# Artemarius/cuda-gaussian-splatting

Hardware: AMD Instinct MI355X
Metric: fwd+bwd Mpixels/s @1080p, 1M Gaussians, SH3 (higher is better)
Workload: dtype f32

## Files before the change

### cuda-gaussian-splatting_amd/csrc/cugs_raster_common.h

```cpp
#pragma once

#include "cugs_gaussian_math.h"

#define CUGS_REC_F4 3

struct RasterGeom {
    int width, height, ntx, ntiles;
    float bg0, bg1, bg2;
};

struct RasterSrc {
    const int32_t* tile_ranges;
    const int32_t* gidx;
    const float* packed;
    const float* means_2d;
    const float* cov_2d_inv;
    const float* rgb;
    const float* opa;
    const uint4* tile_order;
};

template <bool PACKED, bool DEPTH = false>
__device__ __forceinline__ int stage_record(const RasterSrc& s, int li, int end, float4* s_rec,
                                            const float* __restrict__ depths = nullptr) {
    if (li >= end) return -1;
    const int g = s.gidx[li];
    float4 r0, r1, r2;
    if (PACKED) {
        const float4* src = reinterpret_cast<const float4*>(s.packed + (int64_t)g * CUGS_PACKED_STRIDE);
        r0 = src[0]; r1 = src[1]; r2 = src[2];
    } else {
        const float a = s.cov_2d_inv[g * 3 + 0], c = s.cov_2d_inv[g * 3 + 2], o = s.opa[g];
        r0 = make_float4(s.means_2d[g * 2 + 0], s.means_2d[g * 2 + 1], a, s.cov_2d_inv[g * 3 + 1]);
        r1 = make_float4(c, o, (o >= (1.0f / 255.0f)) ? logf(255.0f * o) : -1.0f, 0.0f);
        r2 = make_float4(s.rgb[g * 3 + 0], 0.0f, s.rgb[g * 3 + 1], s.rgb[g * 3 + 2]);
    }
    r1.w = __int_as_float(g);
    if (DEPTH) r2.y = depths[g];
    s_rec[threadIdx.x * CUGS_REC_F4 + 0] = r0;
    s_rec[threadIdx.x * CUGS_REC_F4 + 1] = r1;
    s_rec[threadIdx.x * CUGS_REC_F4 + 2] = r2;
    return g;
}

__device__ __forceinline__ bool may_touch_quad(float4 r0, float4 r1, float qx0, float qy0,
                                               float wx, float wy) {
    const float mx = r0.x, my = r0.y, a = r0.z, b = r0.w, c = r1.x;
    const float tau = r1.z;
    if (!(tau >= 0.0f)) return false;
    if (!(a > 0.0f && c > 0.0f)) return true;
    const float ia = __builtin_amdgcn_rcpf(a), ic = __builtin_amdgcn_rcpf(c);
    const float lx = qx0 - mx, hx = lx + wx, ly = qy0 - my, hy = ly + wy;
    const bool inside = (lx <= 0.0f) && (hx >= 0.0f) && (ly <= 0.0f) && (hy >= 0.0f);
    float X, Y;
    asm("v_max_f32_e64 %0, -%1, %2" : "=v"(X) : "v"(lx), "v"(hx));
    asm("v_max_f32_e64 %0, -%1, %2" : "=v"(Y) : "v"(ly), "v"(hy));
    const float B = a * X * X + 2.0f * fabsf(b) * X * Y + c * Y * Y;
    const float b2 = b + b;
    const float xe = (lx > 0.0f) ? lx : hx, ye = (ly > 0.0f) ? ly : hy;
    const float yv = __builtin_amdgcn_fmed3f(-b * xe * ic, ly, hy);
    const float xv = __builtin_amdgcn_fmed3f(-b * ye * ia, lx, hx);
    const float qx = a * xe * xe + b2 * xe * yv + c * yv * yv;
    const float qy = a * xv * xv + b2 * xv * ye + c * ye * ye;
    const bool out_x = !((lx <= 0.0f) && (hx >= 0.0f)), out_y = !((ly <= 0.0f) && (hy >= 0.0f));
    const float qmin = inside ? 0.0f : fminf(out_x ? qx : 3.0e38f, out_y ? qy : 3.0e38f);
    return !(0.5f * qmin > tau * 1.01f + 0.05f + 4e-6f * B);
}

struct ActiveRect { float x0, y0, wx, wy; };
__device__ __forceinline__ ActiveRect active_rect(unsigned long long active, float quad_cx, float quad_cy) {
    unsigned cols = (unsigned)active | (unsigned)(active >> 32);
    cols |= cols >> 16;
    cols |= cols >> 8;
    cols &= 0xFFu;
    const int x0 = __builtin_ctz(cols), x1 = 31 - __builtin_clz(cols);
    const int y0 = __builtin_ctzll(active) >> 3, y1 = (63 - __builtin_clzll(active)) >> 3;
    return ActiveRect{quad_cx + (float)x0, quad_cy + (float)y0, (float)(x1 - x0), (float)(y1 - y0)};
}

struct PixelEval { float dx, dy, gx, gy, e; };
__device__ __forceinline__ float pixel_alpha_raw(float pxf, float pyf, float mx, float my, float a, float b,
                                                 float c, float o, float open, PixelEval& r) {
    r.dx = pxf - mx;
    r.dy = pyf - my;
    r.gx = fmaf(a, r.dx, b * r.dy);
    r.gy = fmaf(b, r.dx, c * r.dy);
    const float q = fmaf(r.dx, r.gx, r.dy * r.gy);
    r.e = cugs_blend_exp_q(q);
    const float gate = fmaf(q, 0x1p127f, 1.0f);
    return __builtin_fminf(__builtin_fminf((o * open) * r.e, 0.99f), gate);
}
__device__ __forceinline__ float pixel_alpha(float pxf, float pyf, float mx, float my, float a, float b,
                                             float c, float o, float open, PixelEval& r) {
    const float alpha = pixel_alpha_raw(pxf, pyf, mx, my, a, b, c, o, open, r);
    return (alpha < (1.0f / 255.0f)) ? 0.0f : alpha;
}


__device__ __forceinline__ float sat_fma(float a, float b, float c) {
    return __builtin_amdgcn_fmed3f(fmaf(a, b, c), 0.0f, 1.0f);
}
__device__ __forceinline__ float sat_add(float a, float b) { return __builtin_amdgcn_fmed3f(a + b, 0.0f, 1.0f); }

#define CUGS_ALPHA_MIN_PRED 0x1.01010p-8f
__device__ __forceinline__ float passes_alpha_min(float x) {
    return sat_fma(x, 0x1p32f, -CUGS_ALPHA_MIN_PRED * 0x1p32f);
}
__device__ __forceinline__ float below_alpha_cap(float x) { return sat_fma(x, -0x1p32f, 0.99f * 0x1p32f); }

__device__ __forceinline__ int reduce9t_slot(int lane) {
    if (lane & 3) return -1;
    const int bank = (lane >> 2) & 3, row = lane >> 4;
    const int perm[4] = {0, 2, 1, 3};
    if (row == 0) return perm[bank];
    if (row == 1) return bank == 3 ? 8 : 4 + perm[bank];
    if (row == 2 && bank == 0) return 7;
    return -1;
}

__device__ __forceinline__ float reduce9t(float cA, float cB, float v2, float v3, float v4, float v5, float v6,
                                          float v8, float v7) {
    float a0, a1, a2, a3, a4, b0, b1, b2, d;
    asm volatile(
        "s_nop 1\n\t"
        "v_add_f32_dpp %0, %10, %9 row_mirror row_mask:0xf bank_mask:0xf\n\t"
        "v_add_f32_dpp %1, %11, %11 row_mirror row_mask:0xf bank_mask:0x3\n\t"
        "v_add_f32_dpp %1, %12, %12 row_mirror row_mask:0xf bank_mask:0xc\n\t"
        "v_add_f32_dpp %2, %13, %13 row_mirror row_mask:0xf bank_mask:0x3\n\t"
        "v_add_f32_dpp %2, %14, %14 row_mirror row_mask:0xf bank_mask:0xc\n\t"
        "v_add_f32_dpp %3, %15, %15 row_mirror row_mask:0xf bank_mask:0x3\n\t"
        "v_add_f32_dpp %3, %16, %16 row_mirror row_mask:0xf bank_mask:0xc\n\t"
        "v_add_f32_dpp %4, %17, %17 row_mirror row_mask:0xf bank_mask:0xf\n\t"
        "v_add_f32_dpp %5, %0, %0 row_half_mirror row_mask:0xf bank_mask:0x5\n\t"
        "v_add_f32_dpp %5, %1, %1 row_half_mirror row_mask:0xf bank_mask:0xa\n\t"
        "v_add_f32_dpp %7, %4, %4 row_half_mirror row_mask:0xf bank_mask:0xf\n\t"
        "v_add_f32_dpp %6, %2, %2 row_half_mirror row_mask:0xf bank_mask:0x5\n\t"
        "v_add_f32_dpp %6, %3, %3 row_half_mirror row_mask:0xf bank_mask:0xa\n\t"
        "v_mov_b32 %8, %7\n\t"
        "s_nop 1\n\t"
        "v_permlane16_swap_b32 %5, %6\n\t"
        "v_permlane16_swap_b32 %7, %8\n\t"
        "v_add_f32 %5, %5, %6\n\t"
        "v_add_f32 %7, %7, %8\n\t"
        "s_nop 1\n\t"
        "v_permlane32_swap_b32 %5, %7\n\t"
        "v_add_f32 %8, %5, %7\n\t"
        "s_nop 1\n\t"
        "v_add_f32_dpp %8, %8, %8 quad_perm:[1,0,3,2] row_mask:0xf bank_mask:0xf\n\t"
        "s_nop 1\n\t"
        "v_add_f32_dpp %8, %8, %8 quad_perm:[2,3,0,1] row_mask:0xf bank_mask:0xf\n\t"
        : "=&v"(a0), "=&v"(a1), "=&v"(a2), "=&v"(a3), "=&v"(a4), "=&v"(b0), "=&v"(b1), "=&v"(b2), "=&v"(d)
        : "v"(cA), "v"(cB), "v"(v2), "v"(v3), "v"(v4), "v"(v5), "v"(v6), "v"(v8), "v"(v7));
    return d;
}

template <int CTRL>
__device__ __forceinline__ float dpp_mov(float v) {
    return __builtin_bit_cast(float, __builtin_amdgcn_update_dpp(0, __builtin_bit_cast(int, v), CTRL, 0xF, 0xF, false));
}
template <int CTRL>
__device__ __forceinline__ float xchg_add(bool side, float a, float b) {
    return (side ? b : a) + dpp_mov<CTRL>(side ? a : b);
}

__device__ __forceinline__ int reduce9r16_slot(int lane) {
    const int r = lane & 15, bank = r >> 2;
    const int perm[4] = {0, 2, 1, 3};
    if ((r & 3) == 0) return perm[bank];
    if ((r & 3) == 2) return bank == 3 ? 8 : 4 + perm[bank];
    if (r == 1) return 7;
    return -1;
}

__device__ __forceinline__ float reduce_r16_tail(float b0, float b1, float b2, int lane) {
    const bool s1 = (lane & 2) != 0, s0 = (lane & 1) != 0;
    const float c0 = xchg_add<0x4E>(s1, b0, b1);
    const float c1 = b2 + dpp_mov<0x4E>(b2);
    return xchg_add<0xB1>(s0, c0, c1);
}

__device__ __forceinline__ float reduce9r16(float cA, float cB, float v2, float v3, float v4, float v5, float v6,
                                            float v8, float v7, int lane) {
    float a0, a1, a2, a3, a4, b0, b1, b2;
    asm volatile(
        "s_nop 1\n\t"
        "v_add_f32_dpp %0, %9, %8 row_mirror row_mask:0xf bank_mask:0xf\n\t"
        "v_add_f32_dpp %1, %10, %10 row_mirror row_mask:0xf bank_mask:0x3\n\t"
        "v_add_f32_dpp %1, %11, %11 row_mirror row_mask:0xf bank_mask:0xc\n\t"
        "v_add_f32_dpp %2, %12, %12 row_mirror row_mask:0xf bank_mask:0x3\n\t"
        "v_add_f32_dpp %2, %13, %13 row_mirror row_mask:0xf bank_mask:0xc\n\t"
        "v_add_f32_dpp %3, %14, %14 row_mirror row_mask:0xf bank_mask:0x3\n\t"
        "v_add_f32_dpp %3, %15, %15 row_mirror row_mask:0xf bank_mask:0xc\n\t"
        "v_add_f32_dpp %4, %16, %16 row_mirror row_mask:0xf bank_mask:0xf\n\t"
        "v_add_f32_dpp %5, %0, %0 row_half_mirror row_mask:0xf bank_mask:0x5\n\t"
        "v_add_f32_dpp %5, %1, %1 row_half_mirror row_mask:0xf bank_mask:0xa\n\t"
        "v_add_f32_dpp %7, %4, %4 row_half_mirror row_mask:0xf bank_mask:0xf\n\t"
        "v_add_f32_dpp %6, %2, %2 row_half_mirror row_mask:0xf bank_mask:0x5\n\t"
        "v_add_f32_dpp %6, %3, %3 row_half_mirror row_mask:0xf bank_mask:0xa\n\t"
        "s_nop 1\n\t"
        : "=&v"(a0), "=&v"(a1), "=&v"(a2), "=&v"(a3), "=&v"(a4), "=&v"(b0), "=&v"(b1), "=&v"(b2)
        : "v"(cA), "v"(cB), "v"(v2), "v"(v3), "v"(v4), "v"(v5), "v"(v6), "v"(v8), "v"(v7));
    return reduce_r16_tail(b0, b1, b2, lane);
}

__device__ __forceinline__ int reduce10r16_slot(int lane) {
    return ((lane & 15) == 9) ? 9 : reduce9r16_slot(lane);
}

__device__ __forceinline__ float reduce10r16(float cA, float cB, float v2, float v3, float v4, float v5, float v6,
                                             float v8, float v7, float v9, int lane) {
    float a0, a1, a2, a3, a4, b0, b1, b2;
    asm volatile(
        "s_nop 1\n\t"
        "v_add_f32_dpp %0, %9, %8 row_mirror row_mask:0xf bank_mask:0xf\n\t"
        "v_add_f32_dpp %1, %10, %10 row_mirror row_mask:0xf bank_mask:0x3\n\t"
        "v_add_f32_dpp %1, %11, %11 row_mirror row_mask:0xf bank_mask:0xc\n\t"
        "v_add_f32_dpp %2, %12, %12 row_mirror row_mask:0xf bank_mask:0x3\n\t"
        "v_add_f32_dpp %2, %13, %13 row_mirror row_mask:0xf bank_mask:0xc\n\t"
        "v_add_f32_dpp %3, %14, %14 row_mirror row_mask:0xf bank_mask:0x3\n\t"
        "v_add_f32_dpp %3, %15, %15 row_mirror row_mask:0xf bank_mask:0xc\n\t"
        "v_add_f32_dpp %4, %16, %16 row_mirror row_mask:0xf bank_mask:0x3\n\t"
        "v_add_f32_dpp %4, %17, %17 row_mirror row_mask:0xf bank_mask:0xc\n\t"
        "v_add_f32_dpp %5, %0, %0 row_half_mirror row_mask:0xf bank_mask:0x5\n\t"
        "v_add_f32_dpp %5, %1, %1 row_half_mirror row_mask:0xf bank_mask:0xa\n\t"
        "v_add_f32_dpp %7, %4, %4 row_half_mirror row_mask:0xf bank_mask:0xf\n\t"
        "v_add_f32_dpp %6, %2, %2 row_half_mirror row_mask:0xf bank_mask:0x5\n\t"
        "v_add_f32_dpp %6, %3, %3 row_half_mirror row_mask:0xf bank_mask:0xa\n\t"
        "s_nop 1\n\t"
        : "=&v"(a0), "=&v"(a1), "=&v"(a2), "=&v"(a3), "=&v"(a4), "=&v"(b0), "=&v"(b1), "=&v"(b2)
        : "v"(cA), "v"(cB), "v"(v2), "v"(v3), "v"(v4), "v"(v5), "v"(v6), "v"(v8), "v"(v7), "v"(v9));
    return reduce_r16_tail(b0, b1, b2, lane);
}

__device__ __forceinline__ int reduce12r16_slot(int lane) {
    const int r = lane & 15;
    if ((r & 3) == 3) return -1;
    return ((r & 1) ? 2 : ((r >> 1) & 1)) + 3 * ((r >> 2) & 1) + 6 * ((r >> 3) & 1);
}

__device__ __forceinline__ float reduce12r16(const float (&v)[12], int lane) {
    const bool s3 = (lane & 8) != 0, s2 = (lane & 4) != 0;
    float u[6], w[3];
#pragma unroll
    for (int k = 0; k < 6; ++k) u[k] = xchg_add<0x140>(s3, v[k], v[k + 6]);
#pragma unroll
    for (int k = 0; k < 3; ++k) w[k] = xchg_add<0x141>(s2, u[k], u[k + 3]);
    return reduce_r16_tail(w[0], w[1], w[2], lane);
}
```

### cuda-gaussian-splatting_amd/csrc/raster_backward.hip

```cpp
#include "cugs_raster_common.h"

#include <cstdlib>

#ifdef CUGS_DEV
bool cugs_dev_backward_stats();
#endif

namespace {

#define CUGS_BWD_HITS 4
#ifndef CUGS_BWD_HSTRIDE
#define CUGS_BWD_HSTRIDE 64
#endif

template <bool PACKED, bool WIDE, bool STATS, bool DEPTH = false>
__global__ __launch_bounds__(CUGS_BLOCK) void k_raster_backward(RasterGeom geo, RasterSrc src,
                                                                const float* __restrict__ dL_dcolor,
                                                                const float* __restrict__ final_T,
                                                                const int32_t* __restrict__ n_contrib,
                                                                float* __restrict__ grad_accum, int64_t stats_row,
                                                                const float* __restrict__ depths,
                                                                const float* __restrict__ dL_ddepth_map,
                                                                const float* __restrict__ dL_dalpha) {
    __shared__ float4 s_rec[CUGS_BLOCK * CUGS_REC_F4];
    __shared__ float2 s_contrib[4][CUGS_BWD_HITS][CUGS_BWD_HSTRIDE];

#ifdef CUGS_DEV
    const bool no_atomics = stats_row == -2;
#else
    constexpr bool no_atomics = false;
#endif
    unsigned tile;
    int range_start, range_end;
    if (src.tile_order) {
        const uint4 rec = src.tile_order[blockIdx.x];
        tile = rec.x; range_start = (int)rec.y; range_end = (int)rec.z;
    } else {
        tile = cugs_blend_tile(blockIdx.x, (unsigned)geo.ntx, (unsigned)(geo.ntiles / geo.ntx));
        range_start = src.tile_ranges[tile * 2 + 0];
        range_end = src.tile_ranges[tile * 2 + 1];
    }
    const int tile_x = (int)(tile % (unsigned)geo.ntx), tile_y = (int)(tile / (unsigned)geo.ntx);
    const int tid = threadIdx.x, wave = tid >> 6, lane = tid & 63;
    const int quad_x = tile_x * CUGS_TILE + (wave & 1) * 8, quad_y = tile_y * CUGS_TILE + (wave >> 1) * 8;
    const int px = quad_x + (lane & 7), py = quad_y + (lane >> 3);
    const bool inside = (px < geo.width) && (py < geo.height);
    const float pxf = (float)px + 0.5f, pyf = (float)py + 0.5f;
    const float qx0 = (float)quad_x + 0.5f, qy0 = (float)quad_y + 0.5f;

    const int num_in_range = range_end - range_start;
    const int num_batches = (num_in_range + CUGS_BLOCK - 1) / CUGS_BLOCK;

    const int pix = py * geo.width + px;
    float T = inside ? final_T[pix] : 0.0f;
    const int max_contrib = inside ? n_contrib[pix] : 0;
    float dC0 = 0.0f, dC1 = 0.0f, dC2 = 0.0f;
    if (inside) {
        dC0 = dL_dcolor[pix * 3 + 0];
        dC1 = dL_dcolor[pix * 3 + 1];
        dC2 = dL_dcolor[pix * 3 + 2];
    }
    float dDp = 0.0f;
    if (DEPTH && inside && dL_ddepth_map) dDp = dL_ddepth_map[pix];
    const int h2 = lane >> 4, g2i = lane & 15;
    const int gx0 = quad_x + (g2i & 1) * 4, gy = quad_y + (g2i >> 1);
    const float px2 = (float)gx0 + 0.5f, py2 = (float)gy + 0.5f;
    const bool side = (lane & 8) != 0;
    float eA[4], eB[4], e2[4], eZ[4];
#pragma unroll
    for (int i = 0; i < 4; ++i) {
        float r = 0.0f, gg = 0.0f, bb = 0.0f, zz = 0.0f;
        if (gx0 + i < geo.width && gy < geo.height) {
            const int pq = gy * geo.width + gx0 + i, q = pq * 3;
            r = dL_dcolor[q + 0]; gg = dL_dcolor[q + 1]; bb = dL_dcolor[q + 2];
            if (DEPTH && dL_ddepth_map) zz = dL_ddepth_map[pq];
        }
        eA[i] = side ? gg : r; eB[i] = side ? r : gg; e2[i] = bb; eZ[i] = zz;
    }
    const int slot2 = DEPTH ? reduce10r16_slot(lane) : reduce9r16_slot(lane);
    const unsigned slot_off = (unsigned)(slot2 < 0 ? 0 : slot2) * 4u;
    unsigned long long hitrecs = 0ull;

    float D = fmaf(dC2, T * geo.bg2, fmaf(dC1, T * geo.bg1, dC0 * (T * geo.bg0)));
    if (DEPTH && inside && dL_dalpha) D = fmaf(-T, dL_dalpha[pix], D);
    float rem = (inside && max_contrib > 0) ? (float)max_contrib : -1.0f;
    float open = (inside && max_contrib > 0) ? 1.0f : 0.0f;
    bool wave_done = (__ballot(open != 0.0f) == 0ull);
    int pending = 0;
    unsigned st_steps = 0, st_contrib = 0, st_lanes = 0, st_batches = 0, st_tested = 0, st_open = 0;

    auto flush = [&](int cnt) {
        const int rec = (int)((hitrecs >> (16 * h2)) & 0xFFFFull);
        const float4* c4 = reinterpret_cast<const float4*>(&s_contrib[wave][h2][g2i * 4]);
        const float4 p01 = c4[0], p23 = c4[1];
        const float2 mean = *reinterpret_cast<const float2*>(&s_rec[rec]);
        const float4 tail = s_rec[rec + 1];
        const float dy = py2 - mean.y;
        const float dx0 = px2 - mean.x, dx1 = dx0 + 1.0f, dx2 = dx0 + 2.0f, dx3 = dx0 + 3.0f;
        float t = p01.y * dx0;
        float A = p01.y, M1 = t, Mxx = t * dx0;
        float RA = p01.x * eA[0], RB = p01.x * eB[0], R2 = p01.x * e2[0];
        t = p01.w * dx1; A += p01.w; M1 += t; Mxx = fmaf(t, dx1, Mxx);
        RA = fmaf(p01.z, eA[1], RA); RB = fmaf(p01.z, eB[1], RB); R2 = fmaf(p01.z, e2[1], R2);
        t = p23.y * dx2; A += p23.y; M1 += t; Mxx = fmaf(t, dx2, Mxx);
        RA = fmaf(p23.x, eA[2], RA); RB = fmaf(p23.x, eB[2], RB); R2 = fmaf(p23.x, e2[2], R2);
        t = p23.w * dx3; A += p23.w; M1 += t; Mxx = fmaf(t, dx3, Mxx);
        RA = fmaf(p23.z, eA[3], RA); RB = fmaf(p23.z, eB[3], RB); R2 = fmaf(p23.z, e2[3], R2);
        const float oA = tail.y * A;
        M1 *= tail.y; Mxx *= tail.y;
        const float M1y = dy * oA, Myy = dy * M1y, Mxy = dy * M1;
        float total;
        if (DEPTH) {
            float RZ = p01.x * eZ[0];
            RZ = fmaf(p01.z, eZ[1], RZ); RZ = fmaf(p23.x, eZ[2], RZ); RZ = fmaf(p23.z, eZ[3], RZ);
            total = reduce10r16(RA, RB, R2, A, M1, M1y, Mxx, Myy, Mxy, RZ, lane);
        } else {
            total = reduce9r16(RA, RB, R2, A, M1, M1y, Mxx, Myy, Mxy, lane);
        }
        if (slot2 >= 0 && h2 < cnt && !no_atomics) {
            const int g = __float_as_int(tail.w);
            if (WIDE) {
                atomicAdd(grad_accum + (int64_t)g * CUGS_GRAD_STRIDE + slot2, total);
            } else {
                const unsigned off = ((unsigned)g << 6) + slot_off;
                atomicAdd(reinterpret_cast<float*>(reinterpret_cast<char*>(grad_accum) + off), total);
            }
        }
    };

    for (int batch = num_batches - 1; batch >= 0; --batch) {
        if (lane == 0) s_contrib[wave][0][0].x = wave_done ? 1.0f : 0.0f;
        __syncthreads();
        if (s_contrib[0][0][0].x * s_contrib[1][0][0].x * s_contrib[2][0][0].x * s_contrib[3][0][0].x != 0.0f) break;

        stage_record<PACKED, DEPTH>(src, range_start + batch * CUGS_BLOCK + tid, range_end, s_rec, depths);
        __syncthreads();

        if (STATS && !wave_done) ++st_batches;
        if (!wave_done) {
            const int batch_count = min(CUGS_BLOCK, num_in_range - batch * CUGS_BLOCK);
            const int nsub = (batch_count + CUGS_WAVE - 1) / CUGS_WAVE;
            for (int sub = nsub - 1; sub >= 0 && !wave_done; --sub) {
                const int j = sub * CUGS_WAVE + lane;
                const ActiveRect ar = active_rect(__ballot(open != 0.0f), qx0, qy0);
                bool hit = false;
                if (j < batch_count)
                    hit = may_touch_quad(s_rec[j * CUGS_REC_F4 + 0], s_rec[j * CUGS_REC_F4 + 1], ar.x0, ar.y0, ar.wx,
                                         ar.wy);
                unsigned long long mask = __ballot(hit);
                if (STATS) st_tested += min(CUGS_WAVE, batch_count - sub * CUGS_WAVE);
                while (mask != 0ull) {
                    if (STATS) ++st_steps;
                    const int bit = 63 - __builtin_clzll(mask);
                    mask &= ~(1ull << bit);
                    const int rec = (sub * CUGS_WAVE + bit) * CUGS_REC_F4;
                    const float4 g0 = s_rec[rec], g1 = s_rec[rec + 1], col = s_rec[rec + 2];
                    const float o = g1.y;

                    PixelEval e;
                    const float alpha = pixel_alpha_raw(pxf, pyf, g0.x, g0.y, g0.z, g0.w, g1.x, o, open, e);
                    const float passf = passes_alpha_min(alpha);
                    rem -= passf;
                    open = sat_add(rem, 1.0f);
                    const float k = passf * open;
                    const float al = alpha * k;
                    const float gk = k * below_alpha_cap(alpha);

                    const float rcp = __builtin_amdgcn_rcpf(1.0f - al);
                    T *= rcp;
                    const float weight = al * T;
                    float G = fmaf(dC2, col.w, fmaf(dC1, col.z, dC0 * col.x));
                    if (DEPTH) G = fmaf(dDp, col.y, G);
                    const float gate = fmaf(T, G, -(rcp * D)) * gk;
                    D = fmaf(weight, G, D);
                    if (STATS) {
                        const unsigned long long lm = __ballot(k != 0.0f);
                        if (lm) { ++st_contrib; st_lanes += __popcll(lm); st_open += __popcll(__ballot(open != 0.0f)); }
                    }
                    s_contrib[wave][pending][lane] = make_float2(weight, gate * e.e);
                    hitrecs = (hitrecs & ~(0xFFFFull << (16 * pending))) | ((unsigned long long)(unsigned)rec << (16 * pending));
                    if (++pending == CUGS_BWD_HITS) {
                        flush(CUGS_BWD_HITS);
                        pending = 0;
                    }
                    if (__ballot(open != 0.0f) == 0ull) { wave_done = true; break; }
                }
            }
            if (pending) {
                flush(pending);
                pending = 0;
            }
        }
    }
    if (STATS && lane == 0) {
        float* st = grad_accum + (int64_t)stats_row * CUGS_GRAD_STRIDE;
        atomicAdd(&st[0], (float)st_steps); atomicAdd(&st[1], (float)st_contrib); atomicAdd(&st[2], (float)st_lanes);
        atomicAdd(&st[3], (float)st_batches); atomicAdd(&st[4], (float)st_tested); atomicAdd(&st[5], (float)num_batches);
        atomicAdd(&st[7], (float)st_open);
    }
}

template <bool PACKED, bool DEPTH = false>
__global__ __launch_bounds__(CUGS_BLOCK) void k_unpack_grads(int64_t n, const float* __restrict__ acc,
                                                             const float* __restrict__ packed,
                                                             const float* __restrict__ cov_2d_inv,
                                                             float* __restrict__ dL_drgb,
                                                             float* __restrict__ dL_dopa,
                                                             float* __restrict__ dL_dmeans,
                                                             float* __restrict__ dL_dcov,
                                                             float* __restrict__ dL_ddepths) {
    const int64_t i = (int64_t)blockIdx.x * CUGS_BLOCK + threadIdx.x;
    if (i >= n) return;
    const float4* row = reinterpret_cast<const float4*>(acc + i * CUGS_GRAD_STRIDE);
    const float4 r0 = row[0], r1 = row[1];
    float r2;
    if (DEPTH) {
        const float2 w89 = *reinterpret_cast<const float2*>(acc + i * CUGS_GRAD_STRIDE + 8);
        r2 = w89.x;
        dL_ddepths[i] = w89.y;
    } else {
        r2 = acc[i * CUGS_GRAD_STRIDE + 8];
    }
    float a, b, c;
    if (PACKED) {
        const float4* rec = reinterpret_cast<const float4*>(packed + i * CUGS_PACKED_STRIDE);
        const float4 p0 = rec[0];
        a = p0.z; b = p0.w; c = rec[1].x;
    } else {
        a = cov_2d_inv[i * 3 + 0]; b = cov_2d_inv[i * 3 + 1]; c = cov_2d_inv[i * 3 + 2];
    }
    dL_drgb[i * 3 + 0] = r0.x; dL_drgb[i * 3 + 1] = r0.y; dL_drgb[i * 3 + 2] = r0.z;
    dL_dopa[i] = r0.w;
    const GradMoments m{r1.x, r1.y, r1.z, r1.w, r2};
    const Grad2D g = grads_from_moments(m, a, b, c);
    dL_dmeans[i * 2 + 0] = g.mx; dL_dmeans[i * 2 + 1] = g.my;
    dL_dcov[i * 3 + 0] = g.a; dL_dcov[i * 3 + 1] = g.b; dL_dcov[i * 3 + 2] = g.c;
}

}

namespace {
int rasterize_backward_impl(int width, int height, const float background_host[3],
                                       const int32_t* tile_ranges, const int32_t* gaussian_indices,
                                       const float* means_2d, const float* cov_2d_inv, const float* rgb,
                                       const float* opacities_act, const float* packed,
                                       const float* dL_dcolor, const float* final_T,
                                       const int32_t* n_contrib, int64_t n, float* grad_accum,
                                       float* dL_drgb, float* dL_dopacity_act, float* dL_dmeans_2d,
                                       float* dL_dcov_2d_inv, bool prezeroed, const uint32_t* tile_order, void* stream,
                                       bool depth_map = false, const float* depths = nullptr,
                                       const float* dL_ddepth_map = nullptr, const float* dL_dalpha = nullptr,
                                       float* dL_ddepths = nullptr) {
    if (width < 0 || height < 0 || n < 0 || !background_host) return CUGS_EINVAL;
    if (n == 0) return 0;
    if (!grad_accum) return CUGS_EINVAL;
    if ((reinterpret_cast<uintptr_t>(grad_accum) & 63u) != 0) return CUGS_EALIGN;
    const int n_soa = (dL_drgb != nullptr) + (dL_dopacity_act != nullptr) + (dL_dmeans_2d != nullptr) +
                      (dL_dcov_2d_inv != nullptr);
    if (n_soa != 0 && n_soa != 4) return CUGS_EINVAL;
    if (depth_map && (n_soa == 4) != (dL_ddepths != nullptr)) return CUGS_EINVAL;
    if (n_soa == 4 && !packed && !cov_2d_inv) return CUGS_EINVAL;
    if (packed && !cugs_aligned16(packed)) return CUGS_EALIGN;
    if (tile_order && !cugs_aligned16(tile_order)) return CUGS_EALIGN;
    hipStream_t st = static_cast<hipStream_t>(stream);
    int64_t rows = n;
#ifdef CUGS_DEV
    const bool stats = cugs_dev_backward_stats();
    if (stats) rows = n + 1;
#endif
    if (!prezeroed || rows != n)
        CUGS_RETURN_IF_HIP(hipMemsetAsync(grad_accum, 0, sizeof(float) * CUGS_GRAD_STRIDE * (size_t)rows, st));

    const int ntx = (width + CUGS_TILE - 1) / CUGS_TILE, nty = (height + CUGS_TILE - 1) / CUGS_TILE;
    if (ntx > 0 && nty > 0 && gaussian_indices) {
        if (!tile_ranges || !dL_dcolor || !final_T || !n_contrib) return CUGS_EINVAL;
        if (!packed && (!means_2d || !cov_2d_inv || !rgb || !opacities_act)) return CUGS_EINVAL;
        if (depth_map && !depths) return CUGS_EINVAL;
        if ((int64_t)width * height > 2147483647ll / 3) return CUGS_EOVERFLOW;
        RasterGeom geo{width, height, ntx, ntx * nty, background_host[0], background_host[1], background_host[2]};
        RasterSrc src{tile_ranges, gaussian_indices, packed, means_2d, cov_2d_inv, rgb, opacities_act, reinterpret_cast<const uint4*>(tile_order)};
        const bool wide = rows > (int64_t(1) << 26);
        int64_t stats_arg = n;
#ifdef CUGS_DEV
        if (const char* e = std::getenv("CUGS_BWD_NO_ATOMICS")) if (e[0] == '1') stats_arg = -2;
#endif
#define CUGS_LAUNCH_BWD(P, W, S)                                                                              \
    hipLaunchKernelGGL((k_raster_backward<P, W, S>), dim3(geo.ntiles), dim3(CUGS_BLOCK), 0, st, geo, src, \
                       dL_dcolor, final_T, n_contrib, grad_accum, stats_arg, nullptr, nullptr, nullptr)
#define CUGS_LAUNCH_BWD_DEPTH(P, W)                                                                                  \
    hipLaunchKernelGGL((k_raster_backward<P, W, false, true>), dim3(geo.ntiles), dim3(CUGS_BLOCK), 0, st, geo, src, \
                       dL_dcolor, final_T, n_contrib, grad_accum, stats_arg, depths, dL_ddepth_map, dL_dalpha)
        if (depth_map) {
            if (packed) {
                if (wide) CUGS_LAUNCH_BWD_DEPTH(true, true); else CUGS_LAUNCH_BWD_DEPTH(true, false);
            } else {
                if (wide) CUGS_LAUNCH_BWD_DEPTH(false, true); else CUGS_LAUNCH_BWD_DEPTH(false, false);
            }
        } else
#ifdef CUGS_DEV
        if (stats) {
            if (packed) CUGS_LAUNCH_BWD(true, true, true); else CUGS_LAUNCH_BWD(false, true, true);
        } else
#endif
        if (packed) {
            if (wide) CUGS_LAUNCH_BWD(true, true, false); else CUGS_LAUNCH_BWD(true, false, false);
        } else {
            if (wide) CUGS_LAUNCH_BWD(false, true, false); else CUGS_LAUNCH_BWD(false, false, false);
        }
#undef CUGS_LAUNCH_BWD
#undef CUGS_LAUNCH_BWD_DEPTH
        CUGS_LAUNCH_CHECK();
    }
    if (n_soa == 4) {
        const dim3 grid((unsigned)((n + CUGS_BLOCK - 1) / CUGS_BLOCK));
#define CUGS_LAUNCH_UNPACK(P, D)                                                                                 \
    hipLaunchKernelGGL((k_unpack_grads<P, D>), grid, dim3(CUGS_BLOCK), 0, st, n, grad_accum, packed, cov_2d_inv, \
                       dL_drgb, dL_dopacity_act, dL_dmeans_2d, dL_dcov_2d_inv, dL_ddepths)
        if (depth_map) {
            if (packed) CUGS_LAUNCH_UNPACK(true, true); else CUGS_LAUNCH_UNPACK(false, true);
        } else {
            if (packed) CUGS_LAUNCH_UNPACK(true, false); else CUGS_LAUNCH_UNPACK(false, false);
        }
#undef CUGS_LAUNCH_UNPACK
        CUGS_LAUNCH_CHECK();
    }
    return 0;
}

}

extern "C" int cugs_rasterize_backward(int width, int height, const float background_host[3],
                                       const int32_t* tile_ranges, const int32_t* gaussian_indices,
                                       const float* means_2d, const float* cov_2d_inv, const float* rgb,
                                       const float* opacities_act, const float* packed,
                                       const float* dL_dcolor, const float* final_T,
                                       const int32_t* n_contrib, int64_t n, float* grad_accum,
                                       float* dL_drgb, float* dL_dopacity_act, float* dL_dmeans_2d,
                                       float* dL_dcov_2d_inv, void* stream) {
    return rasterize_backward_impl(width, height, background_host, tile_ranges, gaussian_indices, means_2d, cov_2d_inv, rgb,
                                   opacities_act, packed, dL_dcolor, final_T, n_contrib, n, grad_accum, dL_drgb,
                                   dL_dopacity_act, dL_dmeans_2d, dL_dcov_2d_inv, false, nullptr, stream);
}

extern "C" int cugs_rasterize_backward_prezeroed(int width, int height, const float background_host[3],
                                                 const int32_t* tile_ranges, const int32_t* gaussian_indices,
                                                 const float* means_2d, const float* cov_2d_inv, const float* rgb,
                                                 const float* opacities_act, const float* packed,
                                                 const float* dL_dcolor, const float* final_T,
                                                 const int32_t* n_contrib, int64_t n, float* grad_accum,
                                                 float* dL_drgb, float* dL_dopacity_act, float* dL_dmeans_2d,
                                                 float* dL_dcov_2d_inv, void* stream) {
    return rasterize_backward_impl(width, height, background_host, tile_ranges, gaussian_indices, means_2d, cov_2d_inv, rgb,
                                   opacities_act, packed, dL_dcolor, final_T, n_contrib, n, grad_accum, dL_drgb,
                                   dL_dopacity_act, dL_dmeans_2d, dL_dcov_2d_inv, true, nullptr, stream);
}

extern "C" int cugs_rasterize_backward_ordered(int width, int height, const float background_host[3],
                                               const int32_t* tile_ranges, const int32_t* gaussian_indices,
                                               const float* means_2d, const float* cov_2d_inv, const float* rgb,
                                               const float* opacities_act, const float* packed,
                                               const float* dL_dcolor, const float* final_T,
                                               const int32_t* n_contrib, int64_t n, float* grad_accum,
                                               float* dL_drgb, float* dL_dopacity_act, float* dL_dmeans_2d,
                                               float* dL_dcov_2d_inv, int prezeroed, const uint32_t* tile_order,
                                               void* stream) {
    return rasterize_backward_impl(width, height, background_host, tile_ranges, gaussian_indices, means_2d, cov_2d_inv, rgb,
                                   opacities_act, packed, dL_dcolor, final_T, n_contrib, n, grad_accum, dL_drgb,
                                   dL_dopacity_act, dL_dmeans_2d, dL_dcov_2d_inv, prezeroed != 0, tile_order, stream);
}

extern "C" int cugs_rasterize_backward_depth(int width, int height, const float background_host[3],
                                             const int32_t* tile_ranges, const int32_t* gaussian_indices,
                                             const float* means_2d, const float* cov_2d_inv, const float* rgb,
                                             const float* opacities_act, const float* packed,
                                             const float* dL_dcolor, const float* final_T,
                                             const int32_t* n_contrib, int64_t n, float* grad_accum,
                                             float* dL_drgb, float* dL_dopacity_act, float* dL_dmeans_2d,
                                             float* dL_dcov_2d_inv, int prezeroed, const uint32_t* tile_order,
                                             const float* depths, const float* dL_ddepth_map, const float* dL_dalpha,
                                             float* dL_ddepths, void* stream) {
    return rasterize_backward_impl(width, height, background_host, tile_ranges, gaussian_indices, means_2d, cov_2d_inv, rgb,
                                   opacities_act, packed, dL_dcolor, final_T, n_contrib, n, grad_accum, dL_drgb,
                                   dL_dopacity_act, dL_dmeans_2d, dL_dcov_2d_inv, prezeroed != 0, tile_order, stream, true,
                                   depths, dL_ddepth_map, dL_dalpha, dL_ddepths);
}

#ifdef CUGS_DEV
namespace {
__global__ void k_dbg_reduce9(const float* __restrict__ in, float* __restrict__ out, int* __restrict__ slots) {
    const int l = threadIdx.x;
    const bool side = (l & 8) != 0;
    const float v0 = in[0 * 64 + l], v1 = in[1 * 64 + l];
    out[l] = reduce9t(side ? v1 : v0, side ? v0 : v1, in[2 * 64 + l], in[3 * 64 + l], in[4 * 64 + l], in[5 * 64 + l],
                      in[6 * 64 + l], in[8 * 64 + l], in[7 * 64 + l]);
    slots[l] = reduce9t_slot(l);
}
__global__ void k_dbg_reduce9r16(const float* __restrict__ in, float* __restrict__ out, int* __restrict__ slots) {
    const int l = threadIdx.x;
    const bool side = (l & 8) != 0;
    const float v0 = in[0 * 64 + l], v1 = in[1 * 64 + l];
    out[l] = reduce9r16(side ? v1 : v0, side ? v0 : v1, in[2 * 64 + l], in[3 * 64 + l], in[4 * 64 + l], in[5 * 64 + l],
                        in[6 * 64 + l], in[8 * 64 + l], in[7 * 64 + l], l);
    slots[l] = reduce9r16_slot(l);
}
__global__ void k_dbg_reduce10r16(const float* __restrict__ in, float* __restrict__ out, int* __restrict__ slots) {
    const int l = threadIdx.x;
    const bool side = (l & 8) != 0;
    const float v0 = in[0 * 64 + l], v1 = in[1 * 64 + l];
    out[l] = reduce10r16(side ? v1 : v0, side ? v0 : v1, in[2 * 64 + l], in[3 * 64 + l], in[4 * 64 + l], in[5 * 64 + l],
                         in[6 * 64 + l], in[8 * 64 + l], in[7 * 64 + l], in[9 * 64 + l], l);
    slots[l] = reduce10r16_slot(l);
}
__global__ void k_dbg_rcp(const float* __restrict__ in, float* __restrict__ out, int n) {
    const int i = blockIdx.x * blockDim.x + threadIdx.x;
    if (i < n) out[i] = __builtin_amdgcn_rcpf(in[i]);
}
__global__ void k_dbg_blend_exp(const float* __restrict__ q, float* __restrict__ out, int n) {
    const int i = blockIdx.x * blockDim.x + threadIdx.x;
    if (i < n) out[i] = cugs_blend_exp_q(q[i]);
}
__global__ void k_dbg_may_touch_quad(int n, const float* __restrict__ in, const unsigned long long* __restrict__ masks,
                                     int* __restrict__ hit, unsigned long long* __restrict__ pass,
                                     float* __restrict__ rect) {
    const int i = blockIdx.x * blockDim.x + threadIdx.x;
    if (i >= n) return;
    const float* c = in + (int64_t)i * 8;
    alignas(16) float rec[CUGS_PACKED_STRIDE];
    write_packed(rec, 0, c[0], c[1], Sym2{c[2], c[3], c[4]}, 0.0f, 0.0f, 0.0f, c[5]);
    const float4 r0 = reinterpret_cast<const float4*>(rec)[0], r1 = reinterpret_cast<const float4*>(rec)[1];
    const int quad_x = (int)c[6], quad_y = (int)c[7];
    const float qx0 = (float)quad_x + 0.5f, qy0 = (float)quad_y + 0.5f;
    const unsigned long long active = masks[i];
    const ActiveRect ar = active_rect(active, qx0, qy0);
    hit[i] = may_touch_quad(r0, r1, ar.x0, ar.y0, ar.wx, ar.wy) ? 1 : 0;
    unsigned long long p = 0ull;
    for (int l = 0; l < 64; ++l) {
        const float pxf = (float)(quad_x + (l & 7)) + 0.5f, pyf = (float)(quad_y + (l >> 3)) + 0.5f;
        const float open = ((active >> l) & 1ull) ? 1.0f : 0.0f;
        PixelEval e;
        const float alpha = pixel_alpha_raw(pxf, pyf, r0.x, r0.y, r0.z, r0.w, r1.x, r1.y, open, e);
        if (passes_alpha_min(alpha) != 0.0f) p |= 1ull << l;
    }
    pass[i] = p;
    rect[(int64_t)i * 4 + 0] = ar.x0 - qx0; rect[(int64_t)i * 4 + 1] = ar.y0 - qy0;
    rect[(int64_t)i * 4 + 2] = ar.wx; rect[(int64_t)i * 4 + 3] = ar.wy;
}
bool g_dev_backward_stats = false;
}
bool cugs_dev_backward_stats() { return g_dev_backward_stats; }
extern "C" int cugsdbg_backward_stats(int on) { g_dev_backward_stats = (on != 0); return 0; }
extern "C" int cugsdbg_reduce9(const float* in, float* out, int* slots, void* stream) {
    hipLaunchKernelGGL(k_dbg_reduce9, dim3(1), dim3(64), 0, static_cast<hipStream_t>(stream), in, out, slots);
    CUGS_LAUNCH_CHECK();
    return 0;
}
extern "C" int cugsdbg_reduce9r16(const float* in, float* out, int* slots, void* stream) {
    hipLaunchKernelGGL(k_dbg_reduce9r16, dim3(1), dim3(64), 0, static_cast<hipStream_t>(stream), in, out, slots);
    CUGS_LAUNCH_CHECK();
    return 0;
}
extern "C" int cugsdbg_reduce10r16(const float* in, float* out, int* slots, void* stream) {
    hipLaunchKernelGGL(k_dbg_reduce10r16, dim3(1), dim3(64), 0, static_cast<hipStream_t>(stream), in, out, slots);
    CUGS_LAUNCH_CHECK();
    return 0;
}
extern "C" int cugsdbg_blend_exp_q(const float* q, float* out, int n, void* stream) {
    hipLaunchKernelGGL(k_dbg_blend_exp, dim3((n + 255) / 256), dim3(256), 0, static_cast<hipStream_t>(stream), q, out, n);
    CUGS_LAUNCH_CHECK();
    return 0;
}
extern "C" int cugsdbg_rcp(const float* in, float* out, int n, void* stream) {
    hipLaunchKernelGGL(k_dbg_rcp, dim3((n + 255) / 256), dim3(256), 0, static_cast<hipStream_t>(stream), in, out, n);
    CUGS_LAUNCH_CHECK();
    return 0;
}
extern "C" int cugsdbg_may_touch_quad(int n, const float* in, const unsigned long long* masks, int* hit,
                                      unsigned long long* pass, float* rect, void* stream) {
    if (n <= 0) return n == 0 ? 0 : CUGS_EINVAL;
    hipLaunchKernelGGL(k_dbg_may_touch_quad, dim3((n + 255) / 256), dim3(256), 0, static_cast<hipStream_t>(stream), n, in,
                       masks, hit, pass, rect);
    CUGS_LAUNCH_CHECK();
    return 0;
}
#endif
```

### cuda-gaussian-splatting_amd/csrc/raster_forward.hip

```cpp
#include "cugs_raster_common.h"

namespace {

template <bool PACKED, bool DEPTH>
__device__ __forceinline__ void raster_forward_tile(RasterGeom geo, RasterSrc src, float* out_color, float* out_final_T,
                                                    int32_t* out_n_contrib, float4* zero_buf, uint32_t zero_vec4,
                                                    const float* depths, float* out_depth) {
    __shared__ float4 s_rec[CUGS_BLOCK * CUGS_REC_F4];
    __shared__ int s_wave_done[4];

    if (zero_buf) {
        const uint32_t per = (zero_vec4 + gridDim.x - 1) / gridDim.x;
        const uint32_t lo = blockIdx.x * per, hi = min(zero_vec4, lo + per);
        for (uint32_t e = lo + threadIdx.x; e < hi; e += CUGS_BLOCK) cugs_stnt(zero_buf + e, make_float4(0.0f, 0.0f, 0.0f, 0.0f));
    }

    unsigned tile;
    int range_start, range_end;
    if (src.tile_order) {
        const uint4 rec = src.tile_order[blockIdx.x];
        tile = rec.x; range_start = (int)rec.y; range_end = (int)rec.z;
    } else {
        tile = cugs_blend_tile(blockIdx.x, (unsigned)geo.ntx, (unsigned)(geo.ntiles / geo.ntx));
        range_start = src.tile_ranges[tile * 2 + 0];
        range_end = src.tile_ranges[tile * 2 + 1];
    }
    const int tile_x = (int)(tile % (unsigned)geo.ntx), tile_y = (int)(tile / (unsigned)geo.ntx);
    const int tid = threadIdx.x, wave = tid >> 6, lane = tid & 63;
    const int quad_x = tile_x * CUGS_TILE + (wave & 1) * 8, quad_y = tile_y * CUGS_TILE + (wave >> 1) * 8;
    const int px = quad_x + (lane & 7), py = quad_y + (lane >> 3);
    const bool inside = (px < geo.width) && (py < geo.height);
    const float pxf = (float)px + 0.5f, pyf = (float)py + 0.5f;
    const float qx0 = (float)quad_x + 0.5f, qy0 = (float)quad_y + 0.5f;

    const int num_in_range = range_end - range_start;
    const int num_batches = (num_in_range + CUGS_BLOCK - 1) / CUGS_BLOCK;

    typedef float v2f __attribute__((ext_vector_type(2)));
    float T = 1.0f, C0 = 0.0f;
    v2f C12 = {0.0f, 0.0f};
    v2f C0Z = {0.0f, 0.0f};
    float count = 0.0f;
    float open = inside ? 1.0f : 0.0f;
    bool wave_done = (__ballot(open != 0.0f) == 0ull);

    for (int batch = 0; batch < num_batches; ++batch) {
        if (lane == 0) s_wave_done[wave] = wave_done ? 1 : 0;
        __syncthreads();
        if (s_wave_done[0] & s_wave_done[1] & s_wave_done[2] & s_wave_done[3]) break;

        stage_record<PACKED, DEPTH>(src, range_start + batch * CUGS_BLOCK + tid, range_end, s_rec, depths);
        __syncthreads();

        if (!wave_done) {
            const int batch_count = min(CUGS_BLOCK, num_in_range - batch * CUGS_BLOCK);
            for (int sub = 0; sub * CUGS_WAVE < batch_count && !wave_done; ++sub) {
                const int j = sub * CUGS_WAVE + lane;
                const ActiveRect ar = active_rect(__ballot(open != 0.0f), qx0, qy0);
                bool hit = false;
                if (j < batch_count)
                    hit = may_touch_quad(s_rec[j * CUGS_REC_F4 + 0], s_rec[j * CUGS_REC_F4 + 1], ar.x0, ar.y0, ar.wx,
                                         ar.wy);
                unsigned long long mask = __ballot(hit);
                while (mask != 0ull) {
                    const float4* rp = s_rec + (sub * CUGS_WAVE + __builtin_ctzll(mask)) * CUGS_REC_F4;
                    mask &= mask - 1ull;
                    const float4 g0 = rp[0], g1 = rp[1], col = rp[2];
                    const float o = g1.y;
                    PixelEval e;
                    const float alpha = pixel_alpha_raw(pxf, pyf, g0.x, g0.y, g0.z, g0.w, g1.x, o, open, e);
                    const float passf = passes_alpha_min(alpha);
                    const float al = alpha * passf;
                    const float weight = al * T;
                    if (DEPTH) C0Z = __builtin_elementwise_fma((v2f){weight, weight}, (v2f){col.x, col.y}, C0Z);
                    else C0 = fmaf(weight, col.x, C0);
                    C12 = __builtin_elementwise_fma((v2f){weight, weight}, (v2f){col.z, col.w}, C12);
                    T *= (1.0f - al);
                    count += passf;
                    open *= passes_alpha_min(T);
                    if (__ballot(open != 0.0f) == 0ull) { wave_done = true; break; }
                }
            }
        }
    }

    if (inside) {
        const int pix = py * geo.width + px;
        if (DEPTH) {
            C0 = C0Z.x;
            out_depth[pix] = fmaf(T, 0.0f, C0Z.y);
        }
        out_color[pix * 3 + 0] = fmaf(T, geo.bg0, C0);
        out_color[pix * 3 + 1] = fmaf(T, geo.bg1, C12.x);
        out_color[pix * 3 + 2] = fmaf(T, geo.bg2, C12.y);
        out_final_T[pix] = T;
        out_n_contrib[pix] = (int)count;
    }
}

template <bool PACKED>
__global__ __launch_bounds__(CUGS_BLOCK) void k_raster_forward(RasterGeom geo, RasterSrc src,
                                                               float* __restrict__ out_color,
                                                               float* __restrict__ out_final_T,
                                                               int32_t* __restrict__ out_n_contrib,
                                                               float4* __restrict__ zero_buf, uint32_t zero_vec4) {
    raster_forward_tile<PACKED, false>(geo, src, out_color, out_final_T, out_n_contrib, zero_buf, zero_vec4, nullptr,
                                       nullptr);
}

template <bool PACKED>
__global__ __launch_bounds__(CUGS_BLOCK) void k_raster_forward_depth(RasterGeom geo, RasterSrc src,
                                                                     float* __restrict__ out_color,
                                                                     float* __restrict__ out_final_T,
                                                                     int32_t* __restrict__ out_n_contrib,
                                                                     float4* __restrict__ zero_buf, uint32_t zero_vec4,
                                                                     const float* __restrict__ depths,
                                                                     float* __restrict__ out_depth) {
    raster_forward_tile<PACKED, true>(geo, src, out_color, out_final_T, out_n_contrib, zero_buf, zero_vec4, depths,
                                      out_depth);
}

}

namespace {
int rasterize_forward_impl(int width, int height, const float background_host[3], const int32_t* tile_ranges,
                           const int32_t* gaussian_indices, const float* means_2d, const float* cov_2d_inv,
                           const float* rgb, const float* opacities_act, const float* packed, float* out_color,
                           float* out_final_T, int32_t* out_n_contrib, void* zero_buf, size_t zero_bytes,
                           const uint32_t* tile_order, void* stream, bool depth_map = false,
                           const float* depths = nullptr, float* out_depth = nullptr) {
    if (width < 0 || height < 0 || !background_host) return CUGS_EINVAL;
    if (zero_bytes && (!zero_buf || (reinterpret_cast<uintptr_t>(zero_buf) & 15u) || (zero_bytes & 15u) ||
                       zero_bytes / 16 > 0xFFFFFFFFull))
        return zero_buf ? CUGS_EALIGN : CUGS_EINVAL;
    const int ntx = (width + CUGS_TILE - 1) / CUGS_TILE, nty = (height + CUGS_TILE - 1) / CUGS_TILE;
    if (ntx == 0 || nty == 0) {
        if (zero_bytes) CUGS_RETURN_IF_HIP(hipMemsetAsync(zero_buf, 0, zero_bytes, static_cast<hipStream_t>(stream)));
        return 0;
    }
    if (!tile_ranges || !out_color || !out_final_T || !out_n_contrib) return CUGS_EINVAL;
    if (depth_map && (!out_depth || (gaussian_indices && !depths))) return CUGS_EINVAL;
    if (gaussian_indices && !packed && (!means_2d || !cov_2d_inv || !rgb || !opacities_act)) return CUGS_EINVAL;
    if (packed && !cugs_aligned16(packed)) return CUGS_EALIGN;
    if (tile_order && !cugs_aligned16(tile_order)) return CUGS_EALIGN;
    if ((int64_t)width * height > 2147483647ll / 3) return CUGS_EOVERFLOW;
    RasterGeom geo{width, height, ntx, ntx * nty, background_host[0], background_host[1], background_host[2]};
    RasterSrc src{tile_ranges, gaussian_indices, packed, means_2d, cov_2d_inv, rgb, opacities_act, reinterpret_cast<const uint4*>(tile_order)};
    hipStream_t st = static_cast<hipStream_t>(stream);
    float4* zb = zero_bytes ? static_cast<float4*>(zero_buf) : nullptr;
    const uint32_t zv = (uint32_t)(zero_bytes / 16);
    if (depth_map) {
        if (packed)
            hipLaunchKernelGGL((k_raster_forward_depth<true>), dim3(geo.ntiles), dim3(CUGS_BLOCK), 0, st, geo, src,
                               out_color, out_final_T, out_n_contrib, zb, zv, depths, out_depth);
        else
            hipLaunchKernelGGL((k_raster_forward_depth<false>), dim3(geo.ntiles), dim3(CUGS_BLOCK), 0, st, geo, src,
                               out_color, out_final_T, out_n_contrib, zb, zv, depths, out_depth);
    } else if (packed) {
        hipLaunchKernelGGL((k_raster_forward<true>), dim3(geo.ntiles), dim3(CUGS_BLOCK), 0, st, geo, src,
                           out_color, out_final_T, out_n_contrib, zb, zv);
    } else {
        hipLaunchKernelGGL((k_raster_forward<false>), dim3(geo.ntiles), dim3(CUGS_BLOCK), 0, st, geo, src,
                           out_color, out_final_T, out_n_contrib, zb, zv);
    }
    CUGS_LAUNCH_CHECK();
    return 0;
}
}

extern "C" int cugs_rasterize_forward(int width, int height, const float background_host[3],
                                      const int32_t* tile_ranges, const int32_t* gaussian_indices,
                                      const float* means_2d, const float* cov_2d_inv, const float* rgb,
                                      const float* opacities_act, const float* packed, float* out_color,
                                      float* out_final_T, int32_t* out_n_contrib, void* stream) {
    return rasterize_forward_impl(width, height, background_host, tile_ranges, gaussian_indices, means_2d, cov_2d_inv, rgb,
                                  opacities_act, packed, out_color, out_final_T, out_n_contrib, nullptr, 0, nullptr, stream);
}

extern "C" int cugs_rasterize_forward_zero(int width, int height, const float background_host[3],
                                           const int32_t* tile_ranges, const int32_t* gaussian_indices,
                                           const float* means_2d, const float* cov_2d_inv, const float* rgb,
                                           const float* opacities_act, const float* packed, float* out_color,
                                           float* out_final_T, int32_t* out_n_contrib, void* zero_buf,
                                           size_t zero_bytes, void* stream) {
    return rasterize_forward_impl(width, height, background_host, tile_ranges, gaussian_indices, means_2d, cov_2d_inv, rgb,
                                  opacities_act, packed, out_color, out_final_T, out_n_contrib, zero_buf, zero_bytes, nullptr, stream);
}

extern "C" int cugs_rasterize_forward_ordered(int width, int height, const float background_host[3],
                                              const int32_t* tile_ranges, const int32_t* gaussian_indices,
                                              const float* means_2d, const float* cov_2d_inv, const float* rgb,
                                              const float* opacities_act, const float* packed, float* out_color,
                                              float* out_final_T, int32_t* out_n_contrib, void* zero_buf,
                                              size_t zero_bytes, const uint32_t* tile_order, void* stream) {
    return rasterize_forward_impl(width, height, background_host, tile_ranges, gaussian_indices, means_2d, cov_2d_inv, rgb,
                                  opacities_act, packed, out_color, out_final_T, out_n_contrib, zero_buf, zero_bytes, tile_order,
                                  stream);
}

extern "C" int cugs_rasterize_forward_depth(int width, int height, const float background_host[3],
                                            const int32_t* tile_ranges, const int32_t* gaussian_indices,
                                            const float* means_2d, const float* cov_2d_inv, const float* rgb,
                                            const float* opacities_act, const float* packed, float* out_color,
                                            float* out_final_T, int32_t* out_n_contrib, void* zero_buf,
                                            size_t zero_bytes, const uint32_t* tile_order, const float* depths,
                                            float* out_depth, void* stream) {
    return rasterize_forward_impl(width, height, background_host, tile_ranges, gaussian_indices, means_2d, cov_2d_inv, rgb,
                                  opacities_act, packed, out_color, out_final_T, out_n_contrib, zero_buf, zero_bytes, tile_order,
                                  stream, true, depths, out_depth);
}
```

Before: 2678.

## Process blended hits in groups of four and raise backward occupancy hint

```diff
diff --git a/cuda-gaussian-splatting_amd/csrc/cugs_raster_common.h b/cuda-gaussian-splatting_amd/csrc/cugs_raster_common.h
--- a/cuda-gaussian-splatting_amd/csrc/cugs_raster_common.h
+++ b/cuda-gaussian-splatting_amd/csrc/cugs_raster_common.h
@@ -78,6 +78,31 @@
     return ActiveRect{quad_cx + (float)x0, quad_cy + (float)y0, (float)(x1 - x0), (float)(y1 - y0)};
 }
 
+#define CUGS_HIT_GROUP 4
+__device__ __forceinline__ unsigned cugs_pop_hit_desc(unsigned long long& mask) {
+    const unsigned bit = 63u - (unsigned)__builtin_clzll(mask);
+    mask &= ~(1ull << bit);
+    return bit;
+}
+__device__ __forceinline__ unsigned cugs_pop_hit_asc(unsigned long long& mask) {
+    const unsigned bit = (unsigned)__builtin_ctzll(mask);
+    mask &= mask - 1ull;
+    return bit;
+}
+__device__ __forceinline__ unsigned long long cugs_pop_hits4_desc(unsigned long long& mask, unsigned rec_base) {
+    const unsigned r0 = rec_base + cugs_pop_hit_desc(mask) * CUGS_REC_F4;
+    const unsigned r1 = rec_base + cugs_pop_hit_desc(mask) * CUGS_REC_F4;
+    const unsigned r2 = rec_base + cugs_pop_hit_desc(mask) * CUGS_REC_F4;
+    const unsigned r3 = rec_base + cugs_pop_hit_desc(mask) * CUGS_REC_F4;
+    return (unsigned long long)(r0 | (r1 << 16)) | ((unsigned long long)(r2 | (r3 << 16)) << 32);
+}
+__device__ __forceinline__ int cugs_hit(unsigned long long hitrecs, int field) {
+    return (int)((hitrecs >> (16 * field)) & 0xFFFFull);
+}
+__device__ __forceinline__ unsigned long long cugs_set_hit(unsigned long long hitrecs, int field, unsigned rec) {
+    return (hitrecs & ~(0xFFFFull << (16 * field))) | ((unsigned long long)rec << (16 * field));
+}
+
 struct PixelEval { float dx, dy, gx, gy, e; };
 __device__ __forceinline__ float pixel_alpha_raw(float pxf, float pyf, float mx, float my, float a, float b,
                                                  float c, float o, float open, PixelEval& r) {
diff --git a/cuda-gaussian-splatting_amd/csrc/raster_backward.hip b/cuda-gaussian-splatting_amd/csrc/raster_backward.hip
--- a/cuda-gaussian-splatting_amd/csrc/raster_backward.hip
+++ b/cuda-gaussian-splatting_amd/csrc/raster_backward.hip
@@ -9,12 +9,14 @@
 namespace {
 
 #define CUGS_BWD_HITS 4
+static_assert(CUGS_BWD_HITS == CUGS_HIT_GROUP, "a hit group is one flush");
 #ifndef CUGS_BWD_HSTRIDE
 #define CUGS_BWD_HSTRIDE 64
 #endif
 
 template <bool PACKED, bool WIDE, bool STATS, bool DEPTH = false>
-__global__ __launch_bounds__(CUGS_BLOCK) void k_raster_backward(RasterGeom geo, RasterSrc src,
+__global__ __launch_bounds__(CUGS_BLOCK) __attribute__((amdgpu_waves_per_eu(DEPTH ? 7 : 8)))
+void k_raster_backward(RasterGeom geo, RasterSrc src,
                                                                 const float* __restrict__ dL_dcolor,
                                                                 const float* __restrict__ final_T,
                                                                 const int32_t* __restrict__ n_contrib,
@@ -128,6 +130,34 @@
         }
     };
 
+    auto step = [&](const int rec, const int slot) __attribute__((always_inline)) {
+        if (STATS) ++st_steps;
+        const float4 g0 = s_rec[rec], g1 = s_rec[rec + 1], col = s_rec[rec + 2];
+        const float o = g1.y;
+
+        PixelEval e;
+        const float alpha = pixel_alpha_raw(pxf, pyf, g0.x, g0.y, g0.z, g0.w, g1.x, o, open, e);
+        const float passf = passes_alpha_min(alpha);
+        rem -= passf;
+        open = sat_add(rem, 1.0f);
+        const float k = passf * open;
+        const float al = alpha * k;
+        const float gk = k * below_alpha_cap(alpha);
+
+        const float rcp = __builtin_amdgcn_rcpf(1.0f - al);
+        T *= rcp;
+        const float weight = al * T;
+        float G = fmaf(dC2, col.w, fmaf(dC1, col.z, dC0 * col.x));
+        if (DEPTH) G = fmaf(dDp, col.y, G);
+        const float gate = fmaf(T, G, -(rcp * D)) * gk;
+        D = fmaf(weight, G, D);
+        if (STATS) {
+            const unsigned long long lm = __ballot(k != 0.0f);
+            if (lm) { ++st_contrib; st_lanes += __popcll(lm); st_open += __popcll(__ballot(open != 0.0f)); }
+        }
+        s_contrib[wave][slot][lane] = make_float2(weight, gate * e.e);
+    };
+
     for (int batch = num_batches - 1; batch >= 0; --batch) {
         if (lane == 0) s_contrib[wave][0][0].x = wave_done ? 1.0f : 0.0f;
         __syncthreads();
@@ -149,44 +179,31 @@
                                          ar.wy);
                 unsigned long long mask = __ballot(hit);
                 if (STATS) st_tested += min(CUGS_WAVE, batch_count - sub * CUGS_WAVE);
-                while (mask != 0ull) {
-                    if (STATS) ++st_steps;
-                    const int bit = 63 - __builtin_clzll(mask);
-                    mask &= ~(1ull << bit);
-                    const int rec = (sub * CUGS_WAVE + bit) * CUGS_REC_F4;
-                    const float4 g0 = s_rec[rec], g1 = s_rec[rec + 1], col = s_rec[rec + 2];
-                    const float o = g1.y;
-
-                    PixelEval e;
-                    const float alpha = pixel_alpha_raw(pxf, pyf, g0.x, g0.y, g0.z, g0.w, g1.x, o, open, e);
-                    const float passf = passes_alpha_min(alpha);
-                    rem -= passf;
-                    open = sat_add(rem, 1.0f);
-                    const float k = passf * open;
-                    const float al = alpha * k;
-                    const float gk = k * below_alpha_cap(alpha);
-
-                    const float rcp = __builtin_amdgcn_rcpf(1.0f - al);
-                    T *= rcp;
-                    const float weight = al * T;
-                    float G = fmaf(dC2, col.w, fmaf(dC1, col.z, dC0 * col.x));
-                    if (DEPTH) G = fmaf(dDp, col.y, G);
-                    const float gate = fmaf(T, G, -(rcp * D)) * gk;
-                    D = fmaf(weight, G, D);
-                    if (STATS) {
-                        const unsigned long long lm = __ballot(k != 0.0f);
-                        if (lm) { ++st_contrib; st_lanes += __popcll(lm); st_open += __popcll(__ballot(open != 0.0f)); }
-                    }
-                    s_contrib[wave][pending][lane] = make_float2(weight, gate * e.e);
-                    hitrecs = (hitrecs & ~(0xFFFFull << (16 * pending))) | ((unsigned long long)(unsigned)rec << (16 * pending));
-                    if (++pending == CUGS_BWD_HITS) {
-                        flush(CUGS_BWD_HITS);
+                const unsigned rec_sub = (unsigned)(sub * CUGS_WAVE * CUGS_REC_F4);
+                while (pending + __popcll(mask) >= CUGS_BWD_HITS) {
+                    if (pending == 0) {
+                        hitrecs = cugs_pop_hits4_desc(mask, rec_sub);
+                    } else {
+                        do hitrecs = cugs_set_hit(hitrecs, pending, rec_sub + cugs_pop_hit_desc(mask) * CUGS_REC_F4);
+                        while (++pending < CUGS_BWD_HITS);
                         pending = 0;
                     }
-                    if (__ballot(open != 0.0f) == 0ull) { wave_done = true; break; }
+                    step(cugs_hit(hitrecs, 0), 0);
+                    step(cugs_hit(hitrecs, 1), 1);
+                    step(cugs_hit(hitrecs, 2), 2);
+                    step(cugs_hit(hitrecs, 3), 3);
+                    const bool closed = (__ballot(open != 0.0f) == 0ull);
+                    flush(CUGS_BWD_HITS);
+                    if (closed) { wave_done = true; mask = 0ull; break; }
+                }
+                while (mask != 0ull) {
+                    hitrecs = cugs_set_hit(hitrecs, pending, rec_sub + cugs_pop_hit_desc(mask) * CUGS_REC_F4);
+                    ++pending;
                 }
             }
             if (pending) {
+                for (int p = 0; p < pending; ++p) step(cugs_hit(hitrecs, p), p);
+                if (__ballot(open != 0.0f) == 0ull) wave_done = true;
                 flush(pending);
                 pending = 0;
             }
diff --git a/cuda-gaussian-splatting_amd/csrc/raster_forward.hip b/cuda-gaussian-splatting_amd/csrc/raster_forward.hip
--- a/cuda-gaussian-splatting_amd/csrc/raster_forward.hip
+++ b/cuda-gaussian-splatting_amd/csrc/raster_forward.hip
@@ -43,6 +43,22 @@
     float count = 0.0f;
     float open = inside ? 1.0f : 0.0f;
     bool wave_done = (__ballot(open != 0.0f) == 0ull);
+
+    auto step = [&](const float4* rp) __attribute__((always_inline)) {
+        const float4 g0 = rp[0], g1 = rp[1], col = rp[2];
+        const float o = g1.y;
+        PixelEval e;
+        const float alpha = pixel_alpha_raw(pxf, pyf, g0.x, g0.y, g0.z, g0.w, g1.x, o, open, e);
+        const float passf = passes_alpha_min(alpha);
+        const float al = alpha * passf;
+        const float weight = al * T;
+        if (DEPTH) C0Z = __builtin_elementwise_fma((v2f){weight, weight}, (v2f){col.x, col.y}, C0Z);
+        else C0 = fmaf(weight, col.x, C0);
+        C12 = __builtin_elementwise_fma((v2f){weight, weight}, (v2f){col.z, col.w}, C12);
+        T *= (1.0f - al);
+        count += passf;
+        open *= passes_alpha_min(T);
+    };
 
     for (int batch = 0; batch < num_batches; ++batch) {
         if (lane == 0) s_wave_done[wave] = wave_done ? 1 : 0;
@@ -62,22 +78,17 @@
                     hit = may_touch_quad(s_rec[j * CUGS_REC_F4 + 0], s_rec[j * CUGS_REC_F4 + 1], ar.x0, ar.y0, ar.wx,
                                          ar.wy);
                 unsigned long long mask = __ballot(hit);
+                const float4* sub_rec = s_rec + sub * CUGS_WAVE * CUGS_REC_F4;
+                while (__popcll(mask) >= CUGS_HIT_GROUP) {
+                    const float4* r0 = sub_rec + cugs_pop_hit_asc(mask) * CUGS_REC_F4;
+                    const float4* r1 = sub_rec + cugs_pop_hit_asc(mask) * CUGS_REC_F4;
+                    const float4* r2 = sub_rec + cugs_pop_hit_asc(mask) * CUGS_REC_F4;
+                    const float4* r3 = sub_rec + cugs_pop_hit_asc(mask) * CUGS_REC_F4;
+                    step(r0); step(r1); step(r2); step(r3);
+                    if (__ballot(open != 0.0f) == 0ull) { wave_done = true; mask = 0ull; break; }
+                }
                 while (mask != 0ull) {
-                    const float4* rp = s_rec + (sub * CUGS_WAVE + __builtin_ctzll(mask)) * CUGS_REC_F4;
-                    mask &= mask - 1ull;
-                    const float4 g0 = rp[0], g1 = rp[1], col = rp[2];
-                    const float o = g1.y;
-                    PixelEval e;
-                    const float alpha = pixel_alpha_raw(pxf, pyf, g0.x, g0.y, g0.z, g0.w, g1.x, o, open, e);
-                    const float passf = passes_alpha_min(alpha);
-                    const float al = alpha * passf;
-                    const float weight = al * T;
-                    if (DEPTH) C0Z = __builtin_elementwise_fma((v2f){weight, weight}, (v2f){col.x, col.y}, C0Z);
-                    else C0 = fmaf(weight, col.x, C0);
-                    C12 = __builtin_elementwise_fma((v2f){weight, weight}, (v2f){col.z, col.w}, C12);
-                    T *= (1.0f - al);
-                    count += passf;
-                    open *= passes_alpha_min(T);
+                    step(sub_rec + cugs_pop_hit_asc(mask) * CUGS_REC_F4);
                     if (__ballot(open != 0.0f) == 0ull) { wave_done = true; break; }
                 }
             }
```

New measurement: 2727 (median of 6 runs). +1.8%, better.
